# yuxng/PoseCNN

Measured on AMD Instinct MI355X. Metric: RGB-D frames/sec (640x480, 21 classes), higher is better.
Workload: dtype f32

## Files before the change

posecnn_amd/csrc/conv_first.hip:

```cpp
#include <cstdlib>

#include "pcnn_device.h"

namespace {

using namespace pcnn;

constexpr int CF_SEG = 128;
constexpr int CF_ROWS = 16;
constexpr int CF_CIN = 3;
constexpr int CF_ROWF = (CF_SEG + 2) * CF_CIN;

typedef float f4 __attribute__((ext_vector_type(4)));

__global__ __launch_bounds__(256) void conv3x3_c3_bias_relu_kernel(
    const float* __restrict__ x, const float* __restrict__ w, const float* __restrict__ bias,
    float* __restrict__ y, int H, int W, int Cout, int relu, int nseg, int nstrip)
{
  __shared__ float s_in[CF_ROWS + 2][CF_ROWF];
  const int tid = threadIdx.x, lane = tid & 63, wave = tid >> 6;
  const int seg = blockIdx.x % nseg;
  const int strip = (blockIdx.x / nseg) % nstrip;
  const int b = blockIdx.x / (nseg * nstrip);
  const int cg = blockIdx.y;
// ... 229 lines not shown
}

template <bool RAW>
__global__ __launch_bounds__(512, 1) void conv12_wino43_fused_kernel(
    const float* __restrict__ x, const float* __restrict__ w1, const float* __restrict__ b1,
    const float* __restrict__ ut2, const float* __restrict__ b2, float* __restrict__ ypool, int H, int W, int nbx,
    int nby, int imgs_per_group, int relu1, int relu2, RawFrames raw, int ut_frag)
{
  __shared__ float s_in[F12_P + 2][F12_INF];
  __shared__ __attribute__((aligned(16))) float s_y[F12_P][F12_P][64];
  __shared__ __attribute__((aligned(16))) float s_v[2][6 * 16 * 64];
  const int tid = threadIdx.x, lane = tid & 63;
  const int wave = __builtin_amdgcn_readfirstlane(tid >> 6);
  const int bx = blockIdx.x % nbx, by = (blockIdx.x / nbx) % nby, b = blockIdx.x / (nbx * nby);
  const int py0 = 16 * by - 1, px0 = 16 * bx - 1;
  const bool is_depth = RAW && (raw.color == nullptr || b >= raw.n_color);
  const int grp = RAW ? ((raw.color != nullptr && is_depth) ? 1 : 0) : b / imgs_per_group;
  w1 += (size_t)grp * 27 * 64;
  b1 += (size_t)grp * 64;
  ut2 += (size_t)grp * 36 * 64 * 64;
  b2 += (size_t)grp * 64;

  const int n16 = lane & 15, kk = lane >> 4, chalf = wave & 1;
  float wb[7][2], bia[2];
  int tapoff[7];
#pragma unroll
  for (int j = 0; j < 7; j++) {
    const int slot = 4 * j + kk, t = slot - 1;
    const int ky = t / 9, rem = t - 9 * ky;
    tapoff[j] = slot == 0 ? 0 : ky * F12_INF + rem;
#pragma unroll
    for (int c2 = 0; c2 < 2; c2++) wb[j][c2] = w1[(size_t)(t < 0 ? 0 : t) * 64 + 32 * chalf + 16 * c2 + n16];
  }
#pragma unroll
  for (int c2 = 0; c2 < 2; c2++) bia[c2] = b1[32 * chalf + 16 * c2 + n16];
  const float bv2 = b2[16 * (wave & 3) + (lane & 15)];
  F12_TS(0);
  {
    constexpr int NWIN = ((F12_P + 2) * F12_INF + 511) / 512;
    float wv_[NWIN];
#pragma unroll
    for (int e = 0; e < NWIN; e++) {
      const int i = tid + 512 * e;
      const int r = i / F12_INF, j = i - r * F12_INF;
      const int iy = py0 - 1 + r, ix = px0 - 1 + j / CF_CIN, ch = j % CF_CIN;
      const bool ok = i < (F12_P + 2) * F12_INF && iy >= 0 && iy < H && ix >= 0 && ix < W;
      const size_t pix = ok ? ((size_t)b * H + iy) * W + ix : (size_t)b * H * W;
      float val;
      if (!RAW) {
        val = x[pix * CF_CIN + (ok ? ch : 0)];
      } else if (!is_depth) {
        val = (float)((double)raw.color[pix * CF_CIN + (ok ? ch : 0)] - raw.mean[ch]);
      } else {
        const int bd = b - (raw.color ? raw.n_color : 0);
        const size_t pixd = ok ? ((size_t)bd * H + iy) * W + ix : (size_t)bd * H * W;
        const float t = fminf(fmaxf(div_rn((float)raw.depth[pixd], 2000.f), 0.f), 1.f) * 255.f;
        val = (float)((double)t - raw.mean[ch]);
      }
      if (!ok) val = 0.f;
      wv_[e] = val;
    }
#pragma unroll
    for (int e = 0; e < NWIN; e++) {
      const int i = tid + 512 * e;
      if (i < (F12_P + 2) * F12_INF) (&s_in[0][0])[i] = wv_[e];
    }
  }
  {
    if (kk == 0) wb[0][0] = wb[0][1] = 0.f;
    const bool interior = py0 >= 0 && py0 + F12_P <= H && px0 >= 0 && px0 + F12_P <= W;
    const float* s_in_f = &s_in[0][0];
    float* s_y_f = &s_y[0][0][0];
    __syncthreads();
    F12_TS(1);
#define F12_LOAD_A(DST, G)                                                                            \
    {                                                                                                 \
      const int q_ = 16 * (G) + n16, qc_ = q_ < F12_P * F12_P ? q_ : F12_P * F12_P - 1;    \
      const int r_ = qc_ / F12_P, c_ = qc_ - F12_P * r_;                                              \
      const int pixb_ = r_ * F12_INF + c_ * CF_CIN;                                                   \
      _Pragma("unroll") for (int j = 0; j < 7; j++) DST[j] = s_in_f[pixb_ + tapoff[j]];               \
      if (kk == 0) DST[0] = 0.f;                  \
    }
    constexpr int NU = 2 * ((F12_P * F12_P + 15) / 16);
    float av[7], an[7];
    F12_LOAD_A(av, wave >> 1)
    for (int u = wave; u < NU; u += 8) {
      const int g = u >> 1;
      if (u + 8 < NU) F12_LOAD_A(an, (u + 8) >> 1)
      v4f12 acc[2];
#pragma unroll
      for (int c2 = 0; c2 < 2; c2++) acc[c2] = (v4f12){0.f, 0.f, 0.f, 0.f};
#pragma unroll
      for (int j = 0; j < 7; j++)
#pragma unroll
        for (int c2 = 0; c2 < 2; c2++) acc[c2] = __builtin_amdgcn_mfma_f32_16x16x4f32(av[j], wb[j][c2], acc[c2], 0, 0, 0);
      const int qo0 = 16 * g + 4 * kk;
      float* dst = s_y_f + qo0 * 64 + 32 * chalf + n16;
      if (interior && g < F12_P * F12_P / 16) {
#pragma unroll
        for (int i = 0; i < 4; i++)
#pragma unroll
          for (int c2 = 0; c2 < 2; c2++) {
            float a = acc[c2][i] + bia[c2];
            if (relu1) a = a > 0.f ? a : 0.f;
            dst[i * 64 + 16 * c2] = a;
          }
      } else {
#pragma unroll
        for (int i = 0; i < 4; i++) {
          const int qo = qo0 + i;
          const int ro = qo / F12_P, co = qo - F12_P * ro;
          const int yy = py0 + ro, xx = px0 + co;
          const bool ok = yy >= 0 && yy < H && xx >= 0 && xx < W;
#pragma unroll
          for (int c2 = 0; c2 < 2; c2++) {
            float a = acc[c2][i] + bia[c2];
            if (relu1) a = a > 0.f ? a : 0.f;
            if (!ok) a = 0.f;
            if (qo < F12_P * F12_P) dst[i * 64 + 16 * c2] = a;
          }
        }
      }
#pragma unroll
      for (int j = 0; j < 7; j++) av[j] = an[j];
    }
#undef F12_LOAD_A
  }
  __syncthreads();

  F12_TS(2);
  const bool consumer = wave < 4;
  const int lr = lane & 15, lk = lane >> 4;
  const int ptid = tid & 255;
  const int tile = ptid >> 4, cq = ptid & 15;
  const int tyy = tile >> 2, txx = tile & 3;
  v4f12 acc[36];
  const float* ub = ut2 + (size_t)(16 * (wave & 3) + lr) * 64 + 4 * lk;
  f4 a0[4], a1[4], q0[4], q1[4];
  const unsigned uoff = (unsigned)((16 * (wave & 3) + lr) * 64 + 4 * lk);
  const unsigned foff = (unsigned)(((wave & 3) * 4) * 256 + lane * 4);
#define F12_LOADB(D0, D1, K, G)                                                                                  \
  if (ut_frag) {                                                                                                 \
    const float* pk_ = ut2 + (size_t)(K) * 4096 + 256 * (G);                                                     \
    D0 = *reinterpret_cast<const f4*>(pk_ + foff);                                                               \
    D1 = *reinterpret_cast<const f4*>(pk_ + 4096 + foff);                                                        \
  } else {                                                                                                       \
    const float* pk_ = ut2 + (size_t)(K) * 4096 + 16 * (G);                                                      \
    D0 = *reinterpret_cast<const f4*>(pk_ + uoff);                                                               \
    D1 = *reinterpret_cast<const f4*>(pk_ + 4096 + uoff);                                                        \
  }
#define F12_LOADA(D0, D1, BUF, J, G)                                                                             \
  { D0 = *reinterpret_cast<const f4*>(&s_v[BUF][((J) * 16 + lr) * 64 + (((4 * (G) + lk) ^ lr) * 4)]);            \
    D1 = *reinterpret_cast<const f4*>(&s_v[BUF][(((J) + 1) * 16 + lr) * 64 + (((4 * (G) + lk) ^ lr) * 4)]); }
#define F12_PRODUCE(XI, BUF)                                                                                    \
  {                                                                                                             \
    typedef float f2p __attribute__((ext_vector_type(2)));                                                      \
    f2p ta[2][6];                                                                                               \
    _Pragma("unroll") for (int hh = 0; hh < 2; hh++) {                                                          \
      f4 d[3][6];                                                                                               \
      _Pragma("unroll") for (int s3 = 0; s3 < 3; s3++)                                                          \
        _Pragma("unroll") for (int r = 0; r < 6; r++)                                                           \
          if (((XI) == 0 && (r == 0 || r == 2 || r == 4)) || ((XI) == 5 && (r == 1 || r == 3 || r == 5)) ||     \
              ((XI) >= 1 && (XI) <= 4 && r >= 1 && r <= 4))                                                     \
            d[s3][r] = *reinterpret_cast<const f4*>(&s_y[4 * tyy + r][4 * txx + 3 * hh + s3][cq * 4]);          \
      __builtin_amdgcn_sched_barrier(0);                                                                        \
      _Pragma("unroll") for (int s3 = 0; s3 < 3; s3++) {                                                        \
        const int s2 = 3 * hh + s3;                                                                             \
        _Pragma("unroll") for (int hf = 0; hf < 2; hf++) {                                                      \
          f2p e_[6];                                                                                            \
          _Pragma("unroll") for (int r = 0; r < 6; r++) e_[r] = hf ? d[s3][r].zw : d[s3][r].xy;                 \
          if ((XI) == 0) ta[hf][s2] = (4.f * e_[0] - 5.f * e_[2]) + e_[4];                                      \
          else if ((XI) == 5) ta[hf][s2] = (4.f * e_[1] - 5.f * e_[3]) + e_[5];                                 \
          else if ((XI) == 1 || (XI) == 2) {                                                                    \
            const f2p a = e_[4] - 4.f * e_[2], b_ = e_[3] - 4.f * e_[1];                                        \
            ta[hf][s2] = (XI) == 1 ? a + b_ : a - b_;                                                           \
          } else {                                                                                              \
            const f2p c = e_[4] - e_[2], e = 2.f * (e_[3] - e_[1]);                                             \
            ta[hf][s2] = (XI) == 3 ? c + e : c - e;                                                             \
          }                                                                                                     \
        }                                                                                                       \
      }                                                                                                         \
      __builtin_amdgcn_sched_barrier(0);                                                                        \
    }                                                                                                           \
    f2p oa[2][6];                                                                                               \
    _Pragma("unroll") for (int hf = 0; hf < 2; hf++) {                                                          \
      const f2p* t_ = ta[hf];                                                                                   \
      oa[hf][0] = (4.f * t_[0] - 5.f * t_[2]) + t_[4];                                                          \
      { const f2p a = t_[4] - 4.f * t_[2], b_ = t_[3] - 4.f * t_[1]; oa[hf][1] = a + b_; oa[hf][2] = a - b_; }  \
      { const f2p c = t_[4] - t_[2], e = 2.f * (t_[3] - t_[1]); oa[hf][3] = c + e; oa[hf][4] = c - e; }         \
      oa[hf][5] = (4.f * t_[1] - 5.f * t_[3]) + t_[5];                                                          \
    }                                                                                                           \
    _Pragma("unroll") for (int j = 0; j < 6; j++)                                                               \
      *reinterpret_cast<f4*>(&s_v[BUF][(j * 16 + tile) * 64 + ((cq ^ tile) * 4)]) =                             \
          (f4){oa[0][j].x, oa[0][j].y, oa[1][j].x, oa[1][j].y};                                                 \
  }
#define F12_PAIR(XI, J, BUF, NK)                                                                                \
  {                                                                                                             \
    if ((J) == 0) { _Pragma("unroll") for (int g_ = 0; g_ < 4; g_++) F12_LOADA(a0[g_], a1[g_], BUF, 0, g_) }    \
    v4f12 ca_ = (v4f12){0.f, 0.f, 0.f, 0.f}, cb_ = ca_;                                                         \
    _Pragma("unroll") for (int g_ = 0; g_ < 4; g_++) {                                                          \
      __builtin_amdgcn_sched_barrier(0);                                                                        \
      _Pragma("unroll") for (int i_ = 0; i_ < 4; i_++) {                                                        \
        ca_ = __builtin_amdgcn_mfma_f32_16x16x4f32(a0[g_][i_], q0[g_][i_], ca_, 0, 0, 0);                       \
        cb_ = __builtin_amdgcn_mfma_f32_16x16x4f32(a1[g_][i_], q1[g_][i_], cb_, 0, 0, 0);                       \
      }                                                                                                         \
      __builtin_amdgcn_sched_barrier(0);                                                                        \
      if ((J) < 4 && !F12_ABL_NO_A) { F12_LOADA(a0[g_], a1[g_], BUF, (J) + 2, g_) }                             \
      if ((NK) >= 0 && (NK) < 36 && !F12_ABL_NO_B) { F12_LOADB(q0[g_], q1[g_], (NK), g_) }                      \
    }                                                                                                           \
    acc[6 * (XI) + (J)] = ca_;                                                                                  \
    acc[6 * (XI) + (J) + 1] = cb_;                                                                              \
  }
#define F12_CONSUME(XI, BUF)                                                                                    \
  F12_PAIR(XI, 0, BUF, 6 * (XI) + 2) F12_PAIR(XI, 2, BUF, 6 * (XI) + 4) F12_PAIR(XI, 4, BUF, 6 * (XI) + 6)
#define F12_STEP(S)                                                                                             \
  if (consumer) { if ((S) >= 1) { F12_CONSUME((S) - 1, ((S) - 1) & 1) } }                                       \
  else { if ((S) <= 5 && !F12_ABL_NO_T) { F12_PRODUCE((S) <= 5 ? (S) : 5, (S) & 1) } }                          \
  F12_TS(10 + 2 * (S)); F12_TSW(11 + 2 * (S), 4);                                                                \
  __syncthreads();
  if (consumer) { _Pragma("unroll") for (int g = 0; g < 4; g++) F12_LOADB(q0[g], q1[g], 0, g) }
  F12_STEP(0) F12_STEP(1) F12_STEP(2) F12_STEP(3) F12_STEP(4) F12_STEP(5) F12_STEP(6)
#undef F12_STEP
#undef F12_CONSUME
#undef F12_PAIR
#undef F12_PRODUCE
#undef F12_LOADA
#undef F12_LOADB

  F12_TS(3);
  float* s_o = &s_v[0][0];
  if (consumer) {
    typedef float f2e __attribute__((ext_vector_type(2)));
    const int co = 16 * wave + lr;
    const float bv = bv2;
#pragma unroll
    for (int ih = 0; ih < 2; ih++) {
      f2e yo[16];
#pragma unroll
      for (int o = 0; o < 16; o++) yo[o] = (f2e){0.f, 0.f};
#pragma unroll
      for (int nu = 0; nu < 6; nu++) {
        const float c0 = nu == 5 ? 0.f : 1.f;
        const float c1 = nu == 1 ? 1.f : nu == 2 ? -1.f : nu == 3 ? 2.f : nu == 4 ? -2.f : 0.f;
        const float c2 = (nu == 1 || nu == 2) ? 1.f : (nu == 3 || nu == 4) ? 4.f : 0.f;
        const float c3 = nu == 1 ? 1.f : nu == 2 ? -1.f : nu == 3 ? 8.f : nu == 4 ? -8.f : nu == 5 ? 1.f : 0.f;
        f2e m_[6], t_[4];
#pragma unroll
        for (int x_ = 0; x_ < 6; x_++) m_[x_] = (f2e){acc[6 * x_ + nu][2 * ih], acc[6 * x_ + nu][2 * ih + 1]};
        {
          const f2e s = m_[1] + m_[2], d = m_[1] - m_[2], S = m_[3] + m_[4], D = m_[3] - m_[4];
          t_[0] = (m_[0] + s) + S;
          t_[1] = __builtin_elementwise_fma((f2e){2.f, 2.f}, D, d);
          t_[2] = __builtin_elementwise_fma((f2e){4.f, 4.f}, S, s);
          t_[3] = __builtin_elementwise_fma((f2e){8.f, 8.f}, D, d) + m_[5];
        }
#pragma unroll
        for (int a_ = 0; a_ < 4; a_++) {
          yo[4 * a_ + 0] = __builtin_elementwise_fma(t_[a_], (f2e){c0, c0}, yo[4 * a_ + 0]);
          yo[4 * a_ + 1] = __builtin_elementwise_fma(t_[a_], (f2e){c1, c1}, yo[4 * a_ + 1]);
          yo[4 * a_ + 2] = __builtin_elementwise_fma(t_[a_], (f2e){c2, c2}, yo[4 * a_ + 2]);
          yo[4 * a_ + 3] = __builtin_elementwise_fma(t_[a_], (f2e){c3, c3}, yo[4 * a_ + 3]);
        }
      }
#pragma unroll
      for (int o = 0; o < 16; o++) {
        f2e val = yo[o] + (f2e){bv, bv};
        if (relu2) { val.x = val.x > 0.f ? val.x : 0.f; val.y = val.y > 0.f ? val.y : 0.f; }
        yo[o] = val;
      }
#pragma unroll
      for (int a2 = 0; a2 < 2; a2++)
#pragma unroll
        for (int e2 = 0; e2 < 2; e2++) {
          f2e p = yo[4 * (2 * a2) + 2 * e2];
          const f2e p1 = yo[4 * (2 * a2) + 2 * e2 + 1], p2 = yo[4 * (2 * a2 + 1) + 2 * e2], p3 = yo[4 * (2 * a2 + 1) + 2 * e2 + 1];
          p.x = p1.x > p.x ? p1.x : p.x; p.y = p1.y > p.y ? p1.y : p.y;
          p.x = p2.x > p.x ? p2.x : p.x; p.y = p2.y > p.y ? p2.y : p.y;
          p.x = p3.x > p.x ? p3.x : p.x; p.y = p3.y > p.y ? p3.y : p.y;
          s_o[((2 * lk + a2) * 8 + (2 * (2 * ih) + e2)) * 64 + co] = p.x;
          s_o[((2 * lk + a2) * 8 + (2 * (2 * ih + 1) + e2)) * 64 + co] = p.y;
        }
    }
  }
  F12_TS(4);
  __syncthreads();
  const int Hp = H >> 1, Wp = W >> 1;
  for (int i = tid; i < 8 * 8 * 16; i += 512) {
    const int c4 = (i & 15) * 4, pxl = (i >> 4) & 7, pyl = i >> 7;
    *reinterpret_cast<f4*>(ypool + (((size_t)b * Hp + 8 * by + pyl) * Wp + 8 * bx + pxl) * 64 + c4) =
        *reinterpret_cast<const f4*>(&s_o[(pyl * 8 + pxl) * 64 + c4]);
  }
  F12_TS(5);
}

}

extern "C" int pcnn_conv3x3_c3_winograd43_fwd(const float* x, const float* weights, const float* bias,
                                              int B, int H, int W, int Cout, int groups, int relu, float* v,
                                              void* stream_)
{
  PCNN_REQUIRE(B >= 1 && H >= 1 && W >= 1, PCNN_EINVAL, "conv3x3_c3_winograd43: bad shape %dx%dx%d", B, H, W);
  PCNN_REQUIRE(groups >= 1 && B % groups == 0, PCNN_EINVAL, "conv3x3_c3_winograd43: batch %d is not a multiple of groups %d", B, groups);
  PCNN_REQUIRE(Cout >= 64 && Cout % 64 == 0, PCNN_EINVAL,
               "conv3x3_c3_winograd43: output channels must be a multiple of 64 (got %d)", Cout);
  PCNN_REQUIRE(x && weights && bias && v, PCNN_ENULL, "conv3x3_c3_winograd43: NULL pointer");
  PCNN_REQUIRE(aligned16(v) && aligned16(weights) && aligned16(bias), PCNN_EINVAL,
               "conv3x3_c3_winograd43: weights, bias and output must be 16-byte aligned");
  hipStream_t stream = (hipStream_t)stream_;
  const int Ht = (H + 3) / 4, Wt = (W + 3) / 4;
  const int nseg = (Wt + FW_TILES - 1) / FW_TILES;
  const long long blocks = (long long)B * Ht * nseg;
  PCNN_REQUIRE(blocks < (1ll << 31), PCNN_EINVAL, "conv3x3_c3_winograd43: grid too large");
  const long long plane = (long long)B * Ht * Wt * Cout;
  const RawFrames none = {nullptr, nullptr, 0, {0.0, 0.0, 0.0}};
  PCNN_LAUNCH((conv3x3_c3_wino43_kernel<false>), dim3((unsigned)blocks, Cout / 64), dim3(256), 0, stream, x,
              weights, bias, v, H, W, Cout, relu, Ht, Wt, nseg, plane, B / groups, none);
  return check_launch("conv3x3_c3_winograd43_fwd");
}

extern "C" int pcnn_conv3x3_c3_winograd43_raw_fwd(const uint8_t* color_bgr, int num_color, const uint16_t* depth, int num_depth,
                                                  const double* pixel_means, const float* weights, const float* bias, int H,
                                                  int W, int Cout, int relu, float* v, void* stream_)
{
  PCNN_REQUIRE(num_color >= 0 && num_depth >= 0 && num_color + num_depth >= 1 && H >= 1 && W >= 1, PCNN_EINVAL,
               "conv3x3_c3_winograd43_raw: bad shape (%d colour + %d depth frames of %dx%d)", num_color, num_depth, H, W);
  PCNN_REQUIRE(Cout >= 64 && Cout % 64 == 0, PCNN_EINVAL,
               "conv3x3_c3_winograd43_raw: output channels must be a multiple of 64 (got %d)", Cout);
  PCNN_REQUIRE((num_color == 0 || color_bgr) && (num_depth == 0 || depth) && pixel_means && weights && bias && v, PCNN_ENULL,
               "conv3x3_c3_winograd43_raw: NULL pointer");
  PCNN_REQUIRE(aligned16(v) && aligned16(weights) && aligned16(bias), PCNN_EINVAL,
               "conv3x3_c3_winograd43_raw: weights, bias and output must be 16-byte aligned");
  PCNN_REQUIRE(pixel_means[0] - pixel_means[0] == 0.0 && pixel_means[1] - pixel_means[1] == 0.0 && pixel_means[2] - pixel_means[2] == 0.0,
               PCNN_EINVAL, "conv3x3_c3_winograd43_raw: pixel_means must be finite");
  PCNN_REQUIRE((reinterpret_cast<uintptr_t>(depth) & 1u) == 0, PCNN_EINVAL, "conv3x3_c3_winograd43_raw: depth must be 2-byte aligned");
  hipStream_t stream = (hipStream_t)stream_;
  const int B = num_color + num_depth;
  const int Ht = (H + 3) / 4, Wt = (W + 3) / 4;
  const int nseg = (Wt + FW_TILES - 1) / FW_TILES;
  const long long blocks = (long long)B * Ht * nseg;
  PCNN_REQUIRE(blocks < (1ll << 31), PCNN_EINVAL, "conv3x3_c3_winograd43_raw: grid too large");
  const long long plane = (long long)B * Ht * Wt * Cout;
  const RawFrames raw = {num_color ? color_bgr : nullptr, num_depth ? depth : nullptr, num_color,
                         {pixel_means[0], pixel_means[1], pixel_means[2]}};
  PCNN_LAUNCH((conv3x3_c3_wino43_kernel<true>), dim3((unsigned)blocks, Cout / 64), dim3(256), 0, stream, (const float*)nullptr,
              weights, bias, v, H, W, Cout, relu, Ht, Wt, nseg, plane, 1, raw);
  return check_launch("conv3x3_c3_winograd43_raw_fwd");
}

extern "C" int pcnn_conv3x3_c3_fwd(const float* x, const float* weights, const float* bias, int B,
                                   int H, int W, int Cout, int relu, float* y, void* stream_)
{
  PCNN_REQUIRE(B >= 1 && H >= 1 && W >= 1, PCNN_EINVAL, "conv3x3_c3: bad shape %dx%dx%d", B, H, W);
  PCNN_REQUIRE(Cout >= 64 && Cout % 64 == 0, PCNN_EINVAL,
               "conv3x3_c3: output channels must be a multiple of 64 (got %d)", Cout);
  PCNN_REQUIRE(x && weights && bias && y, PCNN_ENULL, "conv3x3_c3: NULL pointer");
  PCNN_REQUIRE(aligned16(y) && aligned16(weights) && aligned16(bias), PCNN_EINVAL,
               "conv3x3_c3: weights, bias and output must be 16-byte aligned");
  hipStream_t stream = (hipStream_t)stream_;
  const int nseg = (W + CF_SEG - 1) / CF_SEG;
  const int nstrip = (H + CF_ROWS - 1) / CF_ROWS;
  const long long blocks = (long long)B * nstrip * nseg;
  PCNN_REQUIRE(blocks < (1ll << 31), PCNN_EINVAL, "conv3x3_c3: grid too large");
  PCNN_LAUNCH(conv3x3_c3_bias_relu_kernel, dim3((unsigned)blocks, Cout / 64), dim3(256), 0, stream,
              x, weights, bias, y, H, W, Cout, relu, nseg, nstrip);
  return check_launch("conv3x3_c3_fwd");
}

static int conv12_check(int B, int H, int W, const void* w1, const void* b1, const void* ut2, const void* b2, const void* y)
{
  PCNN_REQUIRE(B >= 1 && H >= 16 && W >= 16 && H % 16 == 0 && W % 16 == 0, PCNN_EINVAL,
               "conv1_1_conv1_2_fused: the frame must be a multiple of 16 in both directions (got %dx%d)", W, H);
  PCNN_REQUIRE(w1 && b1 && ut2 && b2 && y, PCNN_ENULL, "conv1_1_conv1_2_fused: NULL pointer");
  PCNN_REQUIRE(aligned16(w1) && aligned16(b1) && aligned16(ut2) && aligned16(b2) && aligned16(y), PCNN_EINVAL,
               "conv1_1_conv1_2_fused: weights, biases and output must be 16-byte aligned");
  PCNN_REQUIRE((long long)B * (H / 16) * (W / 16) < (1ll << 31), PCNN_EINVAL, "conv1_1_conv1_2_fused: grid too large");
  return PCNN_OK;
}

extern "C" int pcnn_conv1_1_conv1_2_fused_fwd(const float* x, const float* w1, const float* b1, const float* ut2, int ut2_layout,
                                              const float* b2, int B, int H, int W, int groups, int relu1, int relu2,
                                              float* y_pool, void* stream_)
{
  PCNN_REQUIRE(ut2_layout == 0 || ut2_layout == 1, PCNN_EINVAL,
               "conv1_1_conv1_2_fused: ut2_layout must be 0 (U^T [36][64][64]) or 1 (fragment-major)");
  int st = conv12_check(B, H, W, w1, b1, ut2, b2, y_pool);
  if (st != PCNN_OK) return st;
  PCNN_REQUIRE(x, PCNN_ENULL, "conv1_1_conv1_2_fused: NULL input");
  PCNN_REQUIRE(groups >= 1 && B % groups == 0, PCNN_EINVAL, "conv1_1_conv1_2_fused: batch %d is not a multiple of groups %d", B, groups);
  hipStream_t stream = (hipStream_t)stream_;
  const RawFrames none = {nullptr, nullptr, 0, {0.0, 0.0, 0.0}};
  PCNN_REQUIRE(groups <= 2, PCNN_EINVAL, "conv1_1_conv1_2_fused: at most two filter sets (got %d)", groups);
  const long long blocks = (long long)B * (H / 16) * (W / 16);
  PCNN_LAUNCH((conv12_wino43_fused_kernel<false>), dim3((unsigned)blocks), dim3(512), 0, stream, x, w1, b1, ut2,
              b2, y_pool, H, W, W / 16, H / 16, B / groups, relu1, relu2, none, ut2_layout);
  return check_launch("conv1_1_conv1_2_fused_fwd");
}

extern "C" int pcnn_conv1_1_conv1_2_fused_raw_fwd(const uint8_t* color_bgr, int num_color, const uint16_t* depth, int num_depth,
                                                  const double* pixel_means, const float* w1, const float* b1, const float* ut2,
                                                  int ut2_layout, const float* b2, int H, int W, int relu1, int relu2, float* y_pool,
                                                  void* stream_)
{
  PCNN_REQUIRE(ut2_layout == 0 || ut2_layout == 1, PCNN_EINVAL,
               "conv1_1_conv1_2_fused_raw: ut2_layout must be 0 (U^T [36][64][64]) or 1 (fragment-major)");
  PCNN_REQUIRE(num_color >= 0 && num_depth >= 0 && num_color + num_depth >= 1, PCNN_EINVAL,
               "conv1_1_conv1_2_fused_raw: bad frame counts (%d colour, %d depth)", num_color, num_depth);
  int st = conv12_check(num_color + num_depth, H, W, w1, b1, ut2, b2, y_pool);
  if (st != PCNN_OK) return st;
  PCNN_REQUIRE((num_color == 0 || color_bgr) && (num_depth == 0 || depth) && pixel_means, PCNN_ENULL, "conv1_1_conv1_2_fused_raw: NULL pointer");
  PCNN_REQUIRE(pixel_means[0] - pixel_means[0] == 0.0 && pixel_means[1] - pixel_means[1] == 0.0 && pixel_means[2] - pixel_means[2] == 0.0,
               PCNN_EINVAL, "conv1_1_conv1_2_fused_raw: pixel_means must be finite");
  PCNN_REQUIRE((reinterpret_cast<uintptr_t>(depth) & 1u) == 0, PCNN_EINVAL, "conv1_1_conv1_2_fused_raw: depth must be 2-byte aligned");
  hipStream_t stream = (hipStream_t)stream_;
  const int B = num_color + num_depth;
  const RawFrames raw = {num_color ? color_bgr : nullptr, num_depth ? depth : nullptr, num_color,
                         {pixel_means[0], pixel_means[1], pixel_means[2]}};
  const long long blocks = (long long)B * (H / 16) * (W / 16);
  PCNN_LAUNCH((conv12_wino43_fused_kernel<true>), dim3((unsigned)blocks), dim3(512), 0, stream, (const float*)nullptr,
              w1, b1, ut2, b2, y_pool, H, W, W / 16, H / 16, 1, relu1, relu2, raw, ut2_layout);
  return check_launch("conv1_1_conv1_2_fused_raw_fwd");
// ... 2 lines not shown
```

posecnn_amd/csrc/wino_mfma.hip:

```cpp
#include <cstdlib>

#include "pcnn_device.h"
#include "mfma_ring.h"

namespace {

using namespace pcnn;

constexpr int WM_BC = 64;
constexpr int WM_KC = 64;
constexpr int WM_LD = 64;
constexpr int WM_NBUF = 3;
constexpr int WM_BT = 32;
constexpr int WM_NW = 4;
constexpr int WM_UB = WM_BC / 4 / WM_NW;

enum : int {
  ABL_NO_BARRIER = 1,
  ABL_NO_DMA = 2,
  ABL_NO_LDS_READS = 4,
  ABL_NO_MFMA = 8,
  ABL_NO_FOLD = 16,
  ABL_NO_EPILOGUE = 32,
  ABL_L2_OPERANDS = 64,
// ... 96 lines not shown
  const unsigned lds0 = (unsigned)(unsigned long long)(__attribute__((address_space(3))) float*)smem;
  unsigned adA[4], adB[4];
#pragma unroll
  for (int j = 0; j < 4; j++) {
    const unsigned chb = ring_chunk_bytes(j, lk, lr);
    adA[j] = lds0 + (unsigned)ra0 * 4u + chb;
    adB[j] = lds0 + (unsigned)(WM_NBUF * WM_BT * WM_LD + rb) * 4u + chb;
  }
#define WM_DSREAD(DST, ADDR, OFF)                                                                     \
  if constexpr (!(ABL & ABL_NO_LDS_READS)) RING_DSREAD_B128(DST, ADDR, OFF);                          \
  else asm volatile("" : "+v"(DST) : "v"(ADDR))
#define WM_READ_AT(SA0, SA1, SB, G0, CUR)                                                             \
  _Pragma("unroll") for (int g_ = 0; g_ < 2; g_++) {                                                  \
    WM_DSREAD(SB[g_], adB[(G0) + g_], (CUR) * (64 * WM_LD * 4));                                      \
    WM_DSREAD(SA0[g_], adA[(G0) + g_], (CUR) * (WM_BT * WM_LD * 4));                                  \
    WM_DSREAD(SA1[g_], adA[(G0) + g_], (CUR) * (WM_BT * WM_LD * 4) + 4096);       \
  }
#define WM_READ(SA0, SA1, SB, G0)                                                                     \
  if constexpr (ABL & ABL_NO_LDS_READS) { WM_READ_AT(SA0, SA1, SB, G0, 0); }    \
  else if (cur == 0) { WM_READ_AT(SA0, SA1, SB, G0, 0); }                                             \
  else if (cur == 1) { WM_READ_AT(SA0, SA1, SB, G0, 1); }                                             \
  else { WM_READ_AT(SA0, SA1, SB, G0, 2); }
  static_assert(WM_NBUF == 3, "WM_READ dispatches over a ring of three buffers");
#define WM_MFMA1(SA0, SA1, SB, G, ACC)                                                                \
  if constexpr (ABL & ABL_NO_MFMA) { asm volatile("" :: "v"(SA0[G]), "v"(SA1[G]), "v"(SB[G])); } else \
  _Pragma("unroll") for (int i_ = 0; i_ < 4; i_++) {                                                  \
    ACC[0] = __builtin_amdgcn_mfma_f32_16x16x4f32(SA0[G][i_], SB[G][i_], ACC[0], 0, 0, 0);            \
    ACC[1] = __builtin_amdgcn_mfma_f32_16x16x4f32(SA1[G][i_], SB[G][i_], ACC[1], 0, 0, 0);            \
  }
#define WM_MFMA(SA0, SA1, SB, ACC)                                                                    \
  WM_MFMA1(SA0, SA1, SB, 0, ACC) WM_MFMA1(SA0, SA1, SB, 1, ACC)
#define WM_MFMA1_Z(SA0, SA1, SB, G, ACC)                                                              \
  if constexpr (ABL & ABL_NO_MFMA) { asm volatile("" :: "v"(SA0[G]), "v"(SA1[G]), "v"(SB[G])); } else { \
    const v4f z_ = (v4f){0.f, 0.f, 0.f, 0.f};                                                         \
    ACC[0] = __builtin_amdgcn_mfma_f32_16x16x4f32(SA0[G][0], SB[G][0], z_, 0, 0, 0);                  \
    ACC[1] = __builtin_amdgcn_mfma_f32_16x16x4f32(SA1[G][0], SB[G][0], z_, 0, 0, 0);                  \
    _Pragma("unroll") for (int i_ = 1; i_ < 4; i_++) {                                                \
      ACC[0] = __builtin_amdgcn_mfma_f32_16x16x4f32(SA0[G][i_], SB[G][i_], ACC[0], 0, 0, 0);          \
      ACC[1] = __builtin_amdgcn_mfma_f32_16x16x4f32(SA1[G][i_], SB[G][i_], ACC[1], 0, 0, 0);          \
    }                                                                                                 \
  }
#define WM_FOLD(NU)                                                                                   \
  if constexpr (!(ABL & ABL_NO_FOLD)) {                                                               \
    const int n_ = (NU);                                                                              \
    const float c0 = n_ == 5 ? 0.f : 1.f;                                                             \
    const float c1 = n_ == 1 ? 1.f : n_ == 2 ? -1.f : n_ == 3 ? 2.f : n_ == 4 ? -2.f : 0.f;           \
    const float c2 = (n_ == 1 || n_ == 2) ? 1.f : (n_ == 3 || n_ == 4) ? 4.f : 0.f;                   \
    const float c3 = n_ == 1 ? 1.f : n_ == 2 ? -1.f : n_ == 3 ? 8.f : n_ == 4 ? -8.f : n_ == 5 ? 1.f : 0.f; \
     \
     \
     \
     \
     \
    _Pragma("unroll") for (int b_ = 0; b_ < 2; b_++)                                                \
      _Pragma("unroll") for (int h_ = 0; h_ < 2; h_++) {                                            \
        v2f m_[6], t_[4];                                                                           \
        _Pragma("unroll") for (int x_ = 0; x_ < 6; x_++) m_[x_] = (v2f){acc[x_][b_][2 * h_], acc[x_][b_][2 * h_ + 1]}; \
        const v2f s_ = m_[1] + m_[2], d_ = m_[1] - m_[2], S_ = m_[3] + m_[4], D_ = m_[3] - m_[4];   \
        t_[0] = (m_[0] + s_) + S_;                                                                  \
        t_[1] = __builtin_elementwise_fma((v2f){2.f, 2.f}, D_, d_);                                 \
        t_[2] = __builtin_elementwise_fma((v2f){4.f, 4.f}, S_, s_);                                 \
        t_[3] = __builtin_elementwise_fma((v2f){8.f, 8.f}, D_, d_) + m_[5];                         \
        _Pragma("unroll") for (int a_ = 0; a_ < 4; a_++) {                                          \
          yo2[b_][h_][4 * a_ + 0] = __builtin_elementwise_fma(t_[a_], (v2f){c0, c0}, yo2[b_][h_][4 * a_ + 0]); \
          yo2[b_][h_][4 * a_ + 1] = __builtin_elementwise_fma(t_[a_], (v2f){c1, c1}, yo2[b_][h_][4 * a_ + 1]); \
          yo2[b_][h_][4 * a_ + 2] = __builtin_elementwise_fma(t_[a_], (v2f){c2, c2}, yo2[b_][h_][4 * a_ + 2]); \
          yo2[b_][h_][4 * a_ + 3] = __builtin_elementwise_fma(t_[a_], (v2f){c3, c3}, yo2[b_][h_][4 * a_ + 3]); \
        }                                                                                           \
      }                                                                                             \
  }

#define WM_STAGE(XI, XP)                                                                              \
  do {                                                                                                \
    if constexpr (ABL & ABL_NO_BARRIER) asm volatile("s_waitcnt vmcnt(4) lgkmcnt(0)" ::: "memory");   \
    else asm volatile("s_waitcnt vmcnt(6) lgkmcnt(0)\n\ts_barrier" ::: "memory");                     \
    WM_READ(xa0, xa1, xb, 0);                                                                         \
    __builtin_amdgcn_sched_barrier(0);    \
    if (kc > 0) { WM_MFMA(ya0, ya1, yb, acc[XI]); }                                                   \
    else if ((XI) > 0) { WM_MFMA(ya0, ya1, yb, acc[XP]); }                                            \
    else if (nu > 0) { WM_MFMA(ya0, ya1, yb, acc[5]); WM_FOLD(nup); }                                 \
    {                                                                                                 \
      const int nb = cur >= 1 ? cur - 1 : 2;            \
      WM_DMA(nb, pvo, puo);                                                                           \
      WM_PF_ADVANCE();                                                                                \
    }                                                                                                 \
    __builtin_amdgcn_sched_barrier(0);                                                                \
    asm volatile("s_waitcnt lgkmcnt(0)" ::: "memory");           \
    __builtin_amdgcn_sched_barrier(0);                                                                \
    if (kc == 0) { WM_MFMA1_Z(xa0, xa1, xb, 0, acc[XI]); }           \
    else { WM_MFMA1(xa0, xa1, xb, 0, acc[XI]); }                                                      \
    __builtin_amdgcn_sched_barrier(0);    \
    WM_READ(ya0, ya1, yb, 2);                                                                         \
    __builtin_amdgcn_sched_barrier(0);                                                                \
    WM_MFMA1(xa0, xa1, xb, 1, acc[XI]);                                                               \
    __builtin_amdgcn_sched_barrier(0);                                                                \
    asm volatile("s_waitcnt lgkmcnt(0)" ::: "memory");    \
    cur = cur == 2 ? 0 : cur + 1;                                                                     \
  } while (0)
  static_assert(2 + WM_UB == 6, "the stage barrier's vmcnt(6) counts the 2 + WM_UB DMA instructions a wave issues per stage");

  int nup = -1;
  for (int nu = 0; nu < 6; nu++) {
    for (int kc = 0; kc < NK; kc++) WM_STAGE(0, 5);
    for (int kc = 0; kc < NK; kc++) WM_STAGE(1, 0);
    for (int kc = 0; kc < NK; kc++) WM_STAGE(2, 1);
    for (int kc = 0; kc < NK; kc++) WM_STAGE(3, 2);
    for (int kc = 0; kc < NK; kc++) WM_STAGE(4, 3);
    for (int kc = 0; kc < NK; kc++) WM_STAGE(5, 4);
    nup = nu;
  }
  asm volatile("s_waitcnt lgkmcnt(0)" ::: "memory");
  __builtin_amdgcn_sched_barrier(0);
  WM_MFMA(ya0, ya1, yb, acc[5]);
  WM_FOLD(5);
  asm volatile("s_waitcnt vmcnt(0)" ::: "memory");
  __syncthreads();
#undef WM_STAGE
#undef WM_READ
#undef WM_READ_AT
#undef WM_DSREAD
#undef WM_MFMA
#undef WM_MFMA1
#undef WM_MFMA1_Z
#undef WM_FOLD
#undef WM_DMA
#undef WM_PF_ADVANCE

  if constexpr (ABL & ABL_EPI_REGS_ONLY) {
    const float bv_ = bv;
    float k_ = 0.f;
#pragma unroll
    for (int b = 0; b < 2; b++)
#pragma unroll
      for (int i = 0; i < 4; i++)
#pragma unroll
        for (int o = 0; o < 16; o++) { float val = YO(b, i, o) + bv_; if (relu) val = val > 0.f ? val : 0.f; k_ += val; }
    if (k_ == 12345.678f) y[tid] = k_;
    return;
  }
  if constexpr (ABL & ABL_NO_EPILOGUE) {
    float k_ = 0.f;
#pragma unroll
    for (int b = 0; b < 2; b++)
#pragma unroll
      for (int i = 0; i < 4; i++)
#pragma unroll
        for (int o = 0; o < 16; o++) k_ += YO(b, i, o);
#pragma unroll
    for (int x_ = 0; x_ < 6; x_++) k_ += acc[x_][0][0] + acc[x_][1][1];
    if (k_ == 12345.678f) y[tid] = k_;
    return;
  }
  const int col = 16 * wave + lr;
#pragma unroll
  for (int b = 0; b < 2; b++)
#pragma unroll
    for (int i = 0; i < 4; i++)
#pragma unroll
      for (int o = 0; o < 16; o++) {
        float val = YO(b, i, o) + bv;
        if (relu) val = val > 0.f ? val : 0.f;
        YO(b, i, o) = val;
      }

  constexpr int SYF = WM_BT * 4 * 64;
  const int wcol = col ^ (16 * lk);
  const int HtWt = Ht * Wt;
  const int bimg0 = (int)(t0 / HtWt);
  const int rem0 = (int)(t0 - (long long)bimg0 * HtWt);
  const int ty0 = rem0 / Wt, tx0 = rem0 - ty0 * Wt;
  const int re = (tid >> 4) & 3, rc4 = (tid & 15) * 4;
  int s_img[8], s_tyx[8];
#pragma unroll
  for (int r = 0; r < 8; r++) {
    const int tl = wave + WM_NW * r;
    const unsigned n = (unsigned)(tx0 + tl), q = n / (unsigned)Wt, tx = n - q * (unsigned)Wt;
    const unsigned m = (unsigned)ty0 + q, q2 = m / (unsigned)Ht, ty = m - q2 * (unsigned)Ht;
    s_img[r] = bimg0 + (int)q2;
    s_tyx[r] = t0 + tl < tend ? (int)(ty | (tx << 16)) : 0xffff;
  }
  if (POOL != 1) {
#pragma unroll
    for (int a = 0; a < 4; a++) {
      float* sY = smem + (a & 1) * SYF;
#pragma unroll
      for (int b = 0; b < 2; b++)
#pragma unroll
        for (int i = 0; i < 4; i++) {
          const int tl = 16 * b + 4 * lk + i;
#pragma unroll
          for (int e = 0; e < 4; e++) sY[(tl * 4 + e) * 64 + wcol] = YO(b, i, 4 * a + e);
        }
      __syncthreads();
#pragma unroll
      for (int r = 0; r < 8; r++) {
        const int tl = wave + WM_NW * r;
        const int ty = s_tyx[r] & 0xffff, tx = s_tyx[r] >> 16;
        const int oy = 4 * ty + a, ox = 4 * tx + re;
        if (oy < H && ox < W) {
          const v4f o4 = *reinterpret_cast<const v4f*>(&sY[(tl * 4 + re) * 64 + (rc4 ^ (16 * ((tl >> 2) & 3)))]);
          if constexpr (ABL & ABL_NO_STORES) { if (o4[0] == 12345.678f) y[tid] = o4[1]; }
          else if constexpr (ABL & ABL_NT_STORES) __builtin_nontemporal_store(o4, reinterpret_cast<v4f*>(y + (((long long)s_img[r] * H + oy) * W + ox) * Cout + cb * WM_BC + rc4));
          else *reinterpret_cast<v4f*>(y + (((long long)s_img[r] * H + oy) * W + ox) * Cout + cb * WM_BC + rc4) = o4;
        }
      }
    }
  }
  if (POOL != 0) {
    float* yp = POOL == 1 ? y : ypool;
    float* sY = smem;
    const int Hp = H / 2, Wp = W / 2;
#pragma unroll
    for (int b = 0; b < 2; b++)
#pragma unroll
      for (int i = 0; i < 4; i++) {
        const int tl = 16 * b + 4 * lk + i;
#pragma unroll
        for (int a2 = 0; a2 < 2; a2++)
#pragma unroll
          for (int e2 = 0; e2 < 2; e2++) {
            float p = YO(b, i, 4 * (2 * a2) + 2 * e2);
            const float p1 = YO(b, i, 4 * (2 * a2) + 2 * e2 + 1), p2 = YO(b, i, 4 * (2 * a2 + 1) + 2 * e2),
                        p3 = YO(b, i, 4 * (2 * a2 + 1) + 2 * e2 + 1);
            p = p1 > p ? p1 : p;
            p = p2 > p ? p2 : p;
            p = p3 > p ? p3 : p;
            sY[(tl * 4 + 2 * a2 + e2) * 64 + wcol] = p;
          }
      }
    __syncthreads();
#pragma unroll
    for (int r = 0; r < 8; r++) {
      const int tl = wave + WM_NW * r;
      const int ty = s_tyx[r] & 0xffff, tx = s_tyx[r] >> 16;
      const int py = 2 * ty + (re >> 1), px = 2 * tx + (re & 1);
      if (py < Hp && px < Wp)
        *reinterpret_cast<v4f*>(yp + (((long long)s_img[r] * Hp + py) * Wp + px) * Cout + cb * WM_BC + rc4) =
            *reinterpret_cast<const v4f*>(&sY[(tl * 4 + re) * 64 + (rc4 ^ (16 * ((tl >> 2) & 3)))]);
    }
  }
}

#undef YO

template <int POOL>
__global__ __launch_bounds__(256) void wino43_splitk_reduce_kernel(
    const float* __restrict__ part, int S, long long stride, const float* __restrict__ bias, int relu,
    float* __restrict__ y, float* __restrict__ ypool, int B, int H, int W, int C, int imgs_per_group)
{
  const int c4n = C >> 2;
  const int Ho = POOL ? H / 2 : H, Wo = POOL ? W / 2 : W;
  const long long total = (long long)B * Ho * Wo * c4n;
  for (long long i = (long long)blockIdx.x * 256 + threadIdx.x; i < total; i += (long long)gridDim.x * 256) {
    const int c4 = (int)(i % c4n) * 4;
    long long r = i / c4n;
    const int ox = (int)(r % Wo); r /= Wo;
    const int oy = (int)(r % Ho);
    const int b = (int)(r / Ho);
    const v4f bv = *reinterpret_cast<const v4f*>(bias + (size_t)(b / imgs_per_group) * C + c4);
    v4f best = (v4f){0.f, 0.f, 0.f, 0.f};
#pragma unroll
    for (int q = 0; q < (POOL ? 4 : 1); q++) {
      const int yy = POOL ? 2 * oy + (q >> 1) : oy, xx = POOL ? 2 * ox + (q & 1) : ox;
      const long long o = (((long long)b * H + yy) * W + xx) * C + c4;
      v4f v = *reinterpret_cast<const v4f*>(part + o);
      for (int s2 = 1; s2 < S; s2++) v += *reinterpret_cast<const v4f*>(part + s2 * stride + o);
      v += bv;
      if (relu) {
#pragma unroll
        for (int e = 0; e < 4; e++) v[e] = v[e] > 0.f ? v[e] : 0.f;
      }
      if (POOL != 1) *reinterpret_cast<v4f*>(y + o) = v;
      if (q == 0) best = v;
      else {
#pragma unroll
        for (int e = 0; e < 4; e++) best[e] = v[e] > best[e] ? v[e] : best[e];
      }
    }
    if (POOL != 0) {
      float* yp = POOL == 1 ? y : ypool;
      *reinterpret_cast<v4f*>(yp + (((long long)b * Ho + oy) * Wo + ox) * C + c4) = best;
    }
  }
}

int wino43_cin_split(long long nbt, int ncb, int Cin)
{
  const int NK = Cin / WM_KC;
  int S = 1;
  if (nbt * ncb >= 128) return 1;
  while (S < 8 && nbt * ncb * S * 2 <= 512 && NK % (2 * S) == 0) S *= 2;
  return S;
}

}

extern "C" int pcnn_winograd43_conv_workspace_bytes(int B, int H, int W, int Cin, int Cout, int groups, size_t* bytes)
{
  PCNN_REQUIRE(bytes, PCNN_ENULL, "winograd43_conv_workspace_bytes: NULL output");
  PCNN_REQUIRE(B >= 1 && H >= 1 && W >= 1 && Cin >= 64 && Cout >= 64 && groups >= 1 && B % groups == 0, PCNN_EINVAL,
               "winograd43_conv_workspace_bytes: bad shape");
  const long long tpg = (long long)B * ((H + 3) / 4) * ((W + 3) / 4) / groups;
  const int S = wino43_cin_split((long long)groups * ((tpg + WM_BT - 1) / WM_BT), Cout / WM_BC, Cin);
  *bytes = S > 1 ? sizeof(float) * ((size_t)S * B * H * W * Cout + (size_t)groups * Cout) : 0;
  return PCNN_OK;
}

extern "C" int pcnn_winograd43_conv_fwd(const float* v, const float* ut, const float* bias, int B, int H,
                                        int W, int Cin, int Cout, int groups, int relu, int pool,
                                        float* y, float* y_pool, void* workspace, size_t workspace_bytes,
                                        void* stream_)
{
  PCNN_REQUIRE(B >= 1 && H >= 1 && W >= 1, PCNN_EINVAL, "winograd43_conv: bad shape %dx%dx%d", B, H, W);
  PCNN_REQUIRE(Cin >= 64 && Cin % 64 == 0, PCNN_EINVAL, "winograd43_conv: input channels must be a multiple of 64 (got %d)", Cin);
  PCNN_REQUIRE(Cout >= 64 && Cout % 64 == 0, PCNN_EINVAL, "winograd43_conv: output channels must be a multiple of 64 (got %d)", Cout);
  PCNN_REQUIRE(pool >= 0 && pool <= 2, PCNN_EINVAL, "winograd43_conv: pool must be 0 (none), 1 (pooled only) or 2 (both)");
  PCNN_REQUIRE(!pool || (H % 2 == 0 && W % 2 == 0), PCNN_EINVAL, "winograd43_conv: pooling needs even height/width");
  PCNN_REQUIRE(groups >= 1 && B % groups == 0, PCNN_EINVAL, "winograd43_conv: batch %d is not a multiple of groups %d", B, groups);
  PCNN_REQUIRE(v && ut && bias && y && (pool != 2 || y_pool), PCNN_ENULL, "winograd43_conv: NULL pointer");
  PCNN_REQUIRE(aligned16(v) && aligned16(ut) && aligned16(bias) && aligned16(y) && (pool != 2 || aligned16(y_pool)), PCNN_EINVAL,
               "winograd43_conv: pointers (v, ut, bias, y, y_pool) must be 16-byte aligned");
  hipStream_t stream = (hipStream_t)stream_;
  const int Ht = (H + 3) / 4, Wt = (W + 3) / 4;
  const long long T = (long long)B * Ht * Wt;
  const long long tpg = T / groups;
  const int ncb = Cout / WM_BC;
  const long long nbt = (long long)groups * ((tpg + WM_BT - 1) / WM_BT);
  const long long blocks = ((nbt + 7) / 8) * 8 * ncb;
  PCNN_REQUIRE(blocks < (1ll << 31), PCNN_EINVAL, "winograd43_conv: grid too large");
  PCNN_REQUIRE(T * Cin < (1ll << 30) && (long long)Cout * Cin < (1ll << 30), PCNN_EINVAL,
               "winograd43_conv: a transform plane of %lld x %d (or %d x %d) floats exceeds the kernel's 32-bit byte offsets", T, Cin, Cout, Cin);
  int S = wino43_cin_split(nbt, ncb, Cin);
  const size_t out_elems = (size_t)B * H * W * Cout;
  if (S > 1 && !(workspace && aligned16(workspace) && workspace_bytes >= sizeof(float) * (S * out_elems + (size_t)groups * Cout))) S = 1;
  static const int env_mode = [] { const char* e = getenv("PCNN_WINO_MODE"); return e ? atoi(e) : -1; }();
  const double u_bytes = 36.0 * Cout * (double)Cin * 4.0 * groups, v_bytes = 36.0 * (double)T * Cin * 4.0;
  int mode = (ncb == 8 && u_bytes > v_bytes) ? 1 : 0;
  if (env_mode >= 0) mode = ((env_mode & 1) && ncb == 8) ? 1 : 0;
  const long long nblocks = (mode & 1) ? 8 * nbt : blocks;
#define WM_GO(P, Y, BIAS, RELU, KS, STRIDE) PCNN_LAUNCH((wino43_mfma_kernel<P>), dim3((unsigned)nblocks, KS), dim3(64 * WM_NW), 0, stream, v, ut, BIAS, Y, y_pool, \
                             H, W, Cin, Cout, Ht, Wt, T, tpg, RELU, (int)nbt, ncb, KS, (long long)(STRIDE), mode)
  if (S == 1) {
    if (pool == 0) WM_GO(0, y, bias, relu, 1, 0); else if (pool == 1) WM_GO(1, y, bias, relu, 1, 0); else WM_GO(2, y, bias, relu, 1, 0);
  } else {
    float* part = static_cast<float*>(workspace);
    WM_GO(0, part, (const float*)nullptr, 0, S, out_elems);
    const long long items = (long long)B * (pool ? (H / 2) * (W / 2) : H * W) * (Cout / 4);
    const unsigned rgrid = (unsigned)((items + 255) / 256 < 65536 ? (items + 255) / 256 : 65536);
    if (pool == 0)
      PCNN_LAUNCH(wino43_splitk_reduce_kernel<0>, dim3(rgrid), dim3(256), 0, stream, part, S, (long long)out_elems, bias, relu, y, y_pool, B, H, W, Cout, B / groups);
    else if (pool == 1)
      PCNN_LAUNCH(wino43_splitk_reduce_kernel<1>, dim3(rgrid), dim3(256), 0, stream, part, S, (long long)out_elems, bias, relu, y, y_pool, B, H, W, Cout, B / groups);
    else
      PCNN_LAUNCH(wino43_splitk_reduce_kernel<2>, dim3(rgrid), dim3(256), 0, stream, part, S, (long long)out_elems, bias, relu, y, y_pool, B, H, W, Cout, B / groups);
  }
  return check_launch("winograd43_conv_fwd");
}
```

Measured before the change: 834.6.

## Reuse Winograd input-transform partials and streamline epilogue stores with buffer ops

```diff
diff --git a/posecnn_amd/csrc/conv_first.hip b/posecnn_amd/csrc/conv_first.hip
--- a/posecnn_amd/csrc/conv_first.hip
+++ b/posecnn_amd/csrc/conv_first.hip
@@ -405,10 +405,16 @@
 #define F12_LOADA(D0, D1, BUF, J, G)                                                                             \
   { D0 = *reinterpret_cast<const f4*>(&s_v[BUF][((J) * 16 + lr) * 64 + (((4 * (G) + lk) ^ lr) * 4)]);            \
     D1 = *reinterpret_cast<const f4*>(&s_v[BUF][(((J) + 1) * 16 + lr) * 64 + (((4 * (G) + lk) ^ lr) * 4)]); }
+  typedef float f2p __attribute__((ext_vector_type(2)));
+  f2p sab[2][2][6], sce[2][2][6];
 #define F12_PRODUCE(XI, BUF)                                                                                    \
   {                                                                                                             \
-    typedef float f2p __attribute__((ext_vector_type(2)));                                                      \
     f2p ta[2][6];                                                                                               \
+    if ((XI) == 2 || (XI) == 4) {                                                                               \
+      _Pragma("unroll") for (int hf = 0; hf < 2; hf++)                                                          \
+        _Pragma("unroll") for (int s2 = 0; s2 < 6; s2++)                                                        \
+          ta[hf][s2] = (XI) == 2 ? sab[0][hf][s2] - sab[1][hf][s2] : sce[0][hf][s2] - sce[1][hf][s2];           \
+    } else                                                                                                      \
     _Pragma("unroll") for (int hh = 0; hh < 2; hh++) {                                                          \
       f4 d[3][6];                                                                                               \
       _Pragma("unroll") for (int s3 = 0; s3 < 3; s3++)                                                          \
@@ -424,12 +430,14 @@
           _Pragma("unroll") for (int r = 0; r < 6; r++) e_[r] = hf ? d[s3][r].zw : d[s3][r].xy;                 \
           if ((XI) == 0) ta[hf][s2] = (4.f * e_[0] - 5.f * e_[2]) + e_[4];                                      \
           else if ((XI) == 5) ta[hf][s2] = (4.f * e_[1] - 5.f * e_[3]) + e_[5];                                 \
-          else if ((XI) == 1 || (XI) == 2) {                                                                    \
+          else if ((XI) == 1) {                                                                                 \
             const f2p a = e_[4] - 4.f * e_[2], b_ = e_[3] - 4.f * e_[1];                                        \
-            ta[hf][s2] = (XI) == 1 ? a + b_ : a - b_;                                                           \
-          } else {                                                                                              \
+            sab[0][hf][s2] = a; sab[1][hf][s2] = b_;                                                            \
+            ta[hf][s2] = a + b_;                                                                                \
+          } else {                                                                                 \
             const f2p c = e_[4] - e_[2], e = 2.f * (e_[3] - e_[1]);                                             \
-            ta[hf][s2] = (XI) == 3 ? c + e : c - e;                                                             \
+            sce[0][hf][s2] = c; sce[1][hf][s2] = e;                                                             \
+            ta[hf][s2] = c + e;                                                                                 \
           }                                                                                                     \
         }                                                                                                       \
       }                                                                                                         \
@@ -518,7 +526,7 @@
 #pragma unroll
       for (int o = 0; o < 16; o++) {
         f2e val = yo[o] + (f2e){bv, bv};
-        if (relu2) { val.x = val.x > 0.f ? val.x : 0.f; val.y = val.y > 0.f ? val.y : 0.f; }
+        if (relu2) { asm("v_max_f32_e32 %0, 0, %0" : "+v"(val.x)); asm("v_max_f32_e32 %0, 0, %0" : "+v"(val.y)); }
         yo[o] = val;
       }
 #pragma unroll
diff --git a/posecnn_amd/csrc/wino_mfma.hip b/posecnn_amd/csrc/wino_mfma.hip
--- a/posecnn_amd/csrc/wino_mfma.hip
+++ b/posecnn_amd/csrc/wino_mfma.hip
@@ -272,33 +272,66 @@
     return;
   }
   const int col = 16 * wave + lr;
-#pragma unroll
-  for (int b = 0; b < 2; b++)
-#pragma unroll
-    for (int i = 0; i < 4; i++)
-#pragma unroll
-      for (int o = 0; o < 16; o++) {
-        float val = YO(b, i, o) + bv;
-        if (relu) val = val > 0.f ? val : 0.f;
-        YO(b, i, o) = val;
-      }
+  {
+    const v2f bv2 = (v2f){bv, bv};
+#pragma unroll
+    for (int b = 0; b < 2; b++)
+#pragma unroll
+      for (int h = 0; h < 2; h++)
+#pragma unroll
+        for (int o = 0; o < 16; o++) yo2[b][h][o] += bv2;
+    if (relu) {
+#pragma unroll
+      for (int b = 0; b < 2; b++)
+#pragma unroll
+        for (int i = 0; i < 4; i++)
+#pragma unroll
+          for (int o = 0; o < 16; o++) {
+            float val = YO(b, i, o);
+            asm("v_max_f32_e32 %0, 0, %0" : "+v"(val));
+            YO(b, i, o) = val;
+          }
+    }
+  }
 
   constexpr int SYF = WM_BT * 4 * 64;
   const int wcol = col ^ (16 * lk);
   const int HtWt = Ht * Wt;
-  const int bimg0 = (int)(t0 / HtWt);
-  const int rem0 = (int)(t0 - (long long)bimg0 * HtWt);
-  const int ty0 = rem0 / Wt, tx0 = rem0 - ty0 * Wt;
+  const unsigned t0u = (unsigned)t0;
+  const int bimg0 = (int)(t0u / (unsigned)HtWt);
+  const int rem0 = (int)(t0u - (unsigned)bimg0 * (unsigned)HtWt);
+  const int ty0 = (int)((unsigned)rem0 / (unsigned)Wt), tx0 = rem0 - ty0 * Wt;
   const int re = (tid >> 4) & 3, rc4 = (tid & 15) * 4;
-  int s_img[8], s_tyx[8];
-#pragma unroll
-  for (int r = 0; r < 8; r++) {
-    const int tl = wave + WM_NW * r;
-    const unsigned n = (unsigned)(tx0 + tl), q = n / (unsigned)Wt, tx = n - q * (unsigned)Wt;
-    const unsigned m = (unsigned)ty0 + q, q2 = m / (unsigned)Ht, ty = m - q2 * (unsigned)Ht;
-    s_img[r] = bimg0 + (int)q2;
-    s_tyx[r] = t0 + tl < tend ? (int)(ty | (tx << 16)) : 0xffff;
-  }
+  const int Wp = W / 2;
+  int s_pix[8], s_rct[8];
+  {
+    int img = bimg0, ty = ty0, tx = tx0 + wave;
+    const int nmine = tend - t0 < WM_BT ? (int)(tend - t0) : WM_BT;
+#pragma unroll
+    for (int r = 0; r < 8; r++) {
+      while (tx >= Wt) { tx -= Wt; if (++ty == Ht) { ty = 0; img++; } }
+      const bool mine = wave + WM_NW * r < nmine;
+      const int rows = !mine ? 0 : H - 4 * ty < 4 ? H - 4 * ty : 4, cols = W - 4 * tx < 4 ? W - 4 * tx : 4;
+      s_pix[r] = (img * H + 4 * ty) * W + 4 * tx;
+      s_rct[r] = rows | cols << 3 | tx << 6;
+      tx += WM_NW;
+    }
+  }
+  const unsigned yoff = (unsigned)((re * Cout + rc4) * 4);
+  unsigned rdb[4];
+#pragma unroll
+  for (int g = 0; g < 4; g++) {
+    rdb[g] = (unsigned)(((wave * 4 + re) * 64 + (rc4 ^ (16 * g))) * 4);
+    asm volatile("" : "+v"(rdb[g]));
+  }
+#define WM_STAGED(SY, R) (*reinterpret_cast<const v4f*>(reinterpret_cast<const char*>(SY) + (R) * (WM_NW * 4 * 64 * 4) + rdb[(R) & 3]))
+  typedef unsigned v4u __attribute__((ext_vector_type(4)));
+#define WM_STORE(PTR, BYTES, OFF, O4)                                                                 \
+  do {                                                                                                \
+    if constexpr (ABL & ABL_NO_STORES) { if ((O4)[0] == 12345.678f) y[tid] = (O4)[1]; }               \
+    else if constexpr (ABL & ABL_NT_STORES) __builtin_nontemporal_store(O4, reinterpret_cast<v4f*>(reinterpret_cast<char*>(PTR) + (OFF))); \
+    else __builtin_amdgcn_raw_buffer_store_b128(__builtin_bit_cast(v4u, O4), __builtin_amdgcn_make_buffer_rsrc(PTR, 0, BYTES, 0x00020000), (int)(OFF), 0, 0); \
+  } while (0)
   if (POOL != 1) {
 #pragma unroll
     for (int a = 0; a < 4; a++) {
@@ -314,14 +347,13 @@
       __syncthreads();
 #pragma unroll
       for (int r = 0; r < 8; r++) {
-        const int tl = wave + WM_NW * r;
-        const int ty = s_tyx[r] & 0xffff, tx = s_tyx[r] >> 16;
-        const int oy = 4 * ty + a, ox = 4 * tx + re;
-        if (oy < H && ox < W) {
-          const v4f o4 = *reinterpret_cast<const v4f*>(&sY[(tl * 4 + re) * 64 + (rc4 ^ (16 * ((tl >> 2) & 3)))]);
-          if constexpr (ABL & ABL_NO_STORES) { if (o4[0] == 12345.678f) y[tid] = o4[1]; }
-          else if constexpr (ABL & ABL_NT_STORES) __builtin_nontemporal_store(o4, reinterpret_cast<v4f*>(y + (((long long)s_img[r] * H + oy) * W + ox) * Cout + cb * WM_BC + rc4));
-          else *reinterpret_cast<v4f*>(y + (((long long)s_img[r] * H + oy) * W + ox) * Cout + cb * WM_BC + rc4) = o4;
+        const int rows = s_rct[r] & 7, cols = (s_rct[r] >> 3) & 7;
+        if (a < rows) {
+          const v4f o4 = WM_STAGED(sY, r);
+          float* dst = y + ((long long)(s_pix[r] + a * W) * Cout + cb * WM_BC);
+          const int bytes = ((cols - 1) * Cout + WM_BC) * 4;
+          if (cols == 4) WM_STORE(dst, bytes, yoff, o4);
+          else if (re < cols) WM_STORE(dst, bytes, yoff, o4);
         }
       }
     }
@@ -329,7 +361,7 @@
   if (POOL != 0) {
     float* yp = POOL == 1 ? y : ypool;
     float* sY = smem;
-    const int Hp = H / 2, Wp = W / 2;
+    const unsigned ypoff = (unsigned)((((re >> 1) * Wp + (re & 1)) * Cout + rc4) * 4);
 #pragma unroll
     for (int b = 0; b < 2; b++)
 #pragma unroll
@@ -351,14 +383,18 @@
     __syncthreads();
 #pragma unroll
     for (int r = 0; r < 8; r++) {
-      const int tl = wave + WM_NW * r;
-      const int ty = s_tyx[r] & 0xffff, tx = s_tyx[r] >> 16;
-      const int py = 2 * ty + (re >> 1), px = 2 * tx + (re & 1);
-      if (py < Hp && px < Wp)
-        *reinterpret_cast<v4f*>(yp + (((long long)s_img[r] * Hp + py) * Wp + px) * Cout + cb * WM_BC + rc4) =
-            *reinterpret_cast<const v4f*>(&sY[(tl * 4 + re) * 64 + (rc4 ^ (16 * ((tl >> 2) & 3)))]);
+      const int rows = s_rct[r] & 7, cols = (s_rct[r] >> 3) & 7, tx = s_rct[r] >> 6;
+      if (rows > 0) {
+        const v4f o4 = WM_STAGED(sY, r);
+        float* dst = yp + ((long long)(s_pix[r] / 4 + tx) * Cout + cb * WM_BC);
+        const int bytes = (((rows / 2 - 1) * Wp + cols / 2 - 1) * Cout + WM_BC) * 4;
+        if (rows == 4 && cols == 4) WM_STORE(dst, bytes, ypoff, o4);
+        else if (2 * (re >> 1) < rows && 2 * (re & 1) < cols) WM_STORE(dst, bytes, ypoff, o4);
+      }
     }
   }
+#undef WM_STORE
+#undef WM_STAGED
 }
 
 #undef YO
@@ -450,6 +486,8 @@
   PCNN_REQUIRE(blocks < (1ll << 31), PCNN_EINVAL, "winograd43_conv: grid too large");
   PCNN_REQUIRE(T * Cin < (1ll << 30) && (long long)Cout * Cin < (1ll << 30), PCNN_EINVAL,
                "winograd43_conv: a transform plane of %lld x %d (or %d x %d) floats exceeds the kernel's 32-bit byte offsets", T, Cin, Cout, Cin);
+  PCNN_REQUIRE((long long)W * Cout < (1ll << 28), PCNN_EINVAL,
+               "winograd43_conv: an output row of %d x %d floats exceeds the kernel's 32-bit byte offsets", W, Cout);
   int S = wino43_cin_split(nbt, ncb, Cin);
   const size_t out_elems = (size_t)B * H * W * Cout;
   if (S > 1 && !(workspace && aligned16(workspace) && workspace_bytes >= sizeof(float) * (S * out_elems + (size_t)groups * Cout))) S = 1;
```

Measured after the change: 841.8 (median of 6 runs). Within noise of the previous version (+0.9%).
